# TIERS/multi-modal-loam

Measured on AMD Instinct MI355X. Metric: scans/s (feature-extract+kNN+10 GN iters) on 16-ring x1800 + Livox 24k fused cloud, higher is better.
Workload: dtype f32/f64; 1 GPU; BASELINE configs[1]: fused VLP-16 16x1800 + Livox Horizon 24000 scan (52800 pts), local map 200000 pts, 1 association pass (thres_dist 25), 10 GN iterations, W=1; resident_slots=8192, stream_lanes=2, distinct_scans=64, map_tiles_touched=43, map_tiles_complete=43, parallelism=scan-sharded x1, device=AMD Radeon Graphics, cus=256

## Files before the change

### multi-modal-loam_amd/csrc/capi.hip

```cpp
#include <math.h>
#include <stdarg.h>
#include <stdio.h>
#include <stdlib.h>
#include <string.h>

#include <algorithm>

#include "mml_internal.h"

int mml_launch_detect_line(mml_ctx* ctx, int n, uint16_t* d_final);

namespace {

constexpr int kPackMaxSlots = 16;
constexpr size_t kStageDoubles = 1u << 22;

double* stage_alloc(mml_ctx* ctx, size_t doubles) {
    if (ctx->stage_cursor + doubles > ctx->h_stage_doubles) {
        mml_sync_all(ctx);
        ctx->stage_cursor = 0;
    }
    double* p = ctx->h_stage + ctx->stage_cursor;
    ctx->stage_cursor += (doubles + 7) & ~size_t(7);
    return p;
}

hipError_t read_settings(mml_ctx* ctx) {
    hipDeviceProp_t prop;
    const hipError_t e = hipGetDeviceProperties(&prop, ctx->device);
    if (e != hipSuccess) return e;
    ctx->cus = prop.multiProcessorCount;
    ctx->n_lanes = 2;
    if (const char* v = getenv("MML_LANES")) {
        const int n = atoi(v);
        if (n >= 1 && n <= mml_ctx::MAX_LANES) ctx->n_lanes = n;
    }
    const auto off = [](const char* name) {
        const char* v = getenv(name);
        return v && atoi(v) == 0;
    };
    ctx->onepass_wanted = !off("MML_ASSIGN_ONEPASS");
    ctx->solve_wide = !off("MML_SOLVE_WIDE");
    ctx->use_graph = getenv("MML_NO_GRAPH") == nullptr;
    ctx->lazy_undistort = !off("MML_LAZY_UNDISTORT");
    return hipSuccess;
}

}

double* mml_stage_alloc(mml_ctx* ctx, size_t doubles) { return stage_alloc(ctx, doubles); }

int mml_refuse(mml_ctx* ctx, int code, const char* fmt, ...) {
    if (ctx) {
        char m[192];
        va_list ap;
        va_start(ap, fmt);
        vsnprintf(m, sizeof(m), fmt, ap);
        va_end(ap);
        ctx->err = m;
    }
    return code;
}

extern "C" {

void mml_config_default(mml_config* cfg, int max_scans) {
    memset(cfg, 0, sizeof(*cfg));
    cfg->max_scans = max_scans;
    cfg->max_velo_points = 16 * 1800;
    cfg->max_livox_points = 24000;
    cfg->n_rings = 16;
    cfg->pitch0_deg = -15.0f;
    cfg->pitch_step_deg = 2.0f;
    cfg->n_livox_lines = 6;
    cfg->near_th = 2.0f;
    cfg->far_th = 50.0f;
    cfg->leaf_corner = 0.4f;
// ... 109 lines not shown
    ALLOC(ctx->seg_flat_n, B * 4);
    ALLOC(ctx->op_agg, B * 2 * MML_SEG_MAX);
    ctx->seg_rstride = (int)((NT >> 6) + 6 * L + 8);
    ALLOC(ctx->seg_rs, B * (size_t)ctx->seg_rstride);
    ALLOC(ctx->seg_rw, B * (size_t)ctx->seg_rstride);
    ALLOC(ctx->ln_curv, B * NT);
    ALLOC(ctx->ln_refl, B * NT);
    ALLOC(ctx->ln_attr, B * NT);
    ALLOC(ctx->sel_scratch, 4 * B * NT + 16 * B * (L + 2) + 64);
    {
        const size_t nblk = ((NV > NL ? NV : NL) + 255) / 256;
        ALLOC(ctx->blk_cnt, B * 2 * nblk * 162);
    }
    ALLOC(ctx->assign_aux, B * 8);
    ALLOC(ctx->brk_queue, B * NT);
    ALLOC(ctx->brk_cnt, 2 * B);
    ALLOC(ctx->queue_off, 2 * ((size_t)B + mml_ctx::MAX_LANES + 1));
    ALLOC(ctx->redo_queue, B * NT);
    ALLOC(ctx->st_exit, B * (NT / 256 + L + 8));
    ALLOC(ctx->vx_big, 2 * B);
    ALLOC(ctx->sel_done, B * L + 8);
    ALLOC(ctx->sel_list, 4 * B * L + 8);
    ALLOC(ctx->sel_list_cnt, 2 * B + 8);
    ALLOC(ctx->crop_cnt, B * ((NT + 255) / 256) * 8);
    ALLOC(ctx->cb_n, B * 2);
    ALLOC(ctx->ln_line, B * NT);
    ALLOC(ctx->ln_label, B * NT);
    ALLOC(ctx->fu_info, B * 8);
    ALLOC(ctx->ft_xyz[0], B * MF);
    ALLOC(ctx->ft_xyz[1], B * MF);
    ALLOC(ctx->ft_n, B * 2);
    ALLOC(ctx->vx_keys, B * (size_t)ctx->VX_CAP);
    ALLOC(ctx->vx_gidx, 2 * B * (size_t)ctx->VX_CAP);
    ALLOC(ctx->lf, B * MF);
    ALLOC(ctx->pf, B * MF);
    ALLOC(ctx->assoc_stats, B * 16);
    ALLOC(ctx->hard_list, B * MF * 2);
    ALLOC(ctx->hard_knn, B * MF * 2 * 10);
    ALLOC(ctx->work_off, 2 * B + 8);
    for (int k = 0; k < 2; ++k) {
        ALLOC(ctx->grid[k].pts, MM);
        ALLOC(ctx->grid[k].cell_start, 4 * MM + 4096 + 2);
        ctx->grid[k].m = 0;
    }
    ALLOC(ctx->map_tmp, 2 * MM);
    ALLOC(ctx->map_keys, MM);
    ALLOC(ctx->map_keys2, MM);
    ALLOC(ctx->map_vals, MM);
    ALLOC(ctx->map_vals2, MM);
    ALLOC(ctx->d_x, B * 6);
    ALLOC(ctx->d_pose_in, B * 64);
    ALLOC(ctx->d_result, B * MML_SOLVE_RESULT);
    ALLOC(ctx->d_summ, B * 8);
    ALLOC(ctx->d_trace, B * 6 * 64);
    ALLOC(ctx->d_rec, B * 32);
    ALLOC(ctx->d_und, B * 8);
    ALLOC(ctx->d_und_par, B * 12);
    ALLOC(ctx->d_extr, 16);
    ALLOC(ctx->d_misc, 64);
#undef ALLOC
    ctx->h_stage_doubles = kStageDoubles;
    if ((e = ctx->fixed.alloc_pinned(&ctx->h_stage, ctx->h_stage_doubles + 8)) != hipSuccess) return fail(e, "ctx->h_stage");
    ctx->stage_cursor = 0;
    if (mml_feature_init(ctx) != MML_OK) return fail(hipErrorUnknown, "mml_feature_init");
    if ((e = hipStreamSynchronize(MML_STREAM(ctx))) != hipSuccess) return fail(e, "hipStreamSynchronize");
    *out = ctx;
// ... 714 lines not shown
    for (int i = 0; i < n; ++i) {
        if (lab[i] == 2) flat[nf++] = i;
        if (lab[i] == 1) sharp[ns++] = i;
        if (flags) flags[i] = fin[i];
    }
    *n_sharp = ns;
    *n_flat = nf;
    return MML_OK;
}

static int undistort_enqueue(mml_ctx* ctx, int first_slot, int count, const double* dR, const double* dt, bool listed_only) {
    double* st = stage_alloc(ctx, 12 * (size_t)count);
    for (int i = 0; i < count; ++i) {
        memcpy(st + 12 * i, dR + 9 * i, sizeof(double) * 9);
        memcpy(st + 12 * i + 9, dt + 3 * i, sizeof(double) * 3);
    }
    double* d_par = ctx->d_pose_in + 64 * (size_t)first_slot;
    MML_HIP(hipMemcpyAsync(d_par, st, sizeof(double) * 12 * count, hipMemcpyHostToDevice, MML_STREAM(ctx)));
    return listed_only ? mml_launch_undistort_listed(ctx, first_slot, count, d_par) : mml_launch_undistort(ctx, first_slot, count, d_par);
}

int mml_undistort(mml_ctx* ctx, int first_slot, int count, const double* dR, const double* dt) {
    CHECK_SLOTS(first_slot, count);
    MML_REQUIRE(dR && dt, MML_ERR_INVALID, "null dR/dt");
    int rc = mml_cloud_settle(ctx, first_slot, count);
    if (rc != MML_OK) return rc;
    return undistort_enqueue(ctx, first_slot, count, dR, dt, false);
}

int mml_downsample(mml_ctx* ctx, int first_slot, int count) {
    CHECK_SLOTS(first_slot, count);
    int rc = mml_cloud_settle(ctx, first_slot, count);
    if (rc != MML_OK) return rc;
    rc = mml_launch_downsample(ctx, first_slot, count);
    if (rc != MML_OK) return rc;
    return mml_downsample_redo_overflow(ctx, first_slot, count, nullptr);
}

int mml_features_download(mml_ctx* ctx, int slot, int kind, float* xyz, int capacity, int* n) {
    CHECK_SLOTS(slot, 1);
    MML_REQUIRE((kind == 0 || kind == 1) && n, MML_ERR_INVALID, "bad kind");
    int h = 0;
    MML_HIP(hipMemcpyAsync(&h, ctx->ft_n + kind * ctx->B + slot, sizeof(int), hipMemcpyDeviceToHost, MML_STREAM(ctx)));
    MML_HIP(hipStreamSynchronize(MML_STREAM(ctx)));
    MML_REQUIRE(h >= 0, MML_ERR_CAPACITY, "down-sample overflowed max_features / voxel capacity");
    *n = h;
    if (!xyz || h == 0) return MML_OK;
    MML_REQUIRE(capacity >= h, MML_ERR_CAPACITY, "download capacity too small");
    std::vector<float4> tmp(h);
    MML_HIP(hipMemcpyAsync(tmp.data(), ctx->ft_xyz[kind] + (size_t)slot * ctx->MF, sizeof(float4) * h,
                           hipMemcpyDeviceToHost, MML_STREAM(ctx)));
    MML_HIP(hipStreamSynchronize(MML_STREAM(ctx)));
    for (int i = 0; i < h; ++i) {
        xyz[3 * i] = tmp[i].x;
        xyz[3 * i + 1] = tmp[i].y;
        xyz[3 * i + 2] = tmp[i].z;
    }
    return MML_OK;
}

int mml_features_upload(mml_ctx* ctx, int slot, int kind, const float* xyz, int n) {
    CHECK_SLOTS(slot, 1);
    MML_REQUIRE((kind == 0 || kind == 1) && n >= 0 && (n == 0 || xyz), MML_ERR_INVALID, "bad arguments");
    MML_REQUIRE(n <= ctx->MF, MML_ERR_CAPACITY, "more features than max_features");
    std::vector<float4> tmp(n ? n : 1);
    for (int i = 0; i < n; ++i) tmp[i] = make_float4(xyz[3 * i], xyz[3 * i + 1], xyz[3 * i + 2], 0.f);
    if (n)
// ... 581 lines not shown
    if (packed) {
        const size_t c = (size_t)count, n = 34 * c + 16;
        double* hp = stage_alloc(ctx, n);
        dp = ctx->d_pose_in + 64 * (size_t)first_slot;
        for (size_t i = 0; i < c; ++i) {
            memcpy(hp + 12 * i, dR + 9 * i, sizeof(double) * 9);
            memcpy(hp + 12 * i + 9, dt + 3 * i, sizeof(double) * 3);
            double q[4];
            so3_exp_h(x_inout + 6 * i + 3, q);
            pose_to_Twl(q, x_inout + 6 * i, T_bl, hp + 12 * c + 16 * i);
        }
        memcpy(hp + 28 * c, x_inout, sizeof(double) * 6 * c);
        memcpy(hp + 34 * c, T_bl, sizeof(double) * 16);
        if (hipMemcpyAsync(dp, hp, sizeof(double) * n, hipMemcpyHostToDevice, MML_STREAM(ctx)) != hipSuccess) return MML_ERR_HIP;
        h_res = stage_alloc(ctx, MML_SOLVE_RESULT * c);
    }
    if (lanes > 1) {
        if (hipEventRecord(ctx->lane_mark[0], ctx->streams[0]) != hipSuccess) return MML_ERR_HIP;
        for (int l = 1; l < mml_ctx::MAX_LANES; ++l)
            if (hipStreamWaitEvent(ctx->streams[l], ctx->lane_mark[0], 0) != hipSuccess) return MML_ERR_HIP;
    }
    auto piece_span = [&](int p, int& f, int& c) {
        f = first_slot + p * chunk;
        c = std::min(chunk, first_slot + count - f);
        return c > 0;
    };
    auto run_stage = [&](int stage, int f, int c) -> int {
        const int off = f - first_slot;
        switch (stage) {
            case 0: return mml_launch_extract(ctx, f, c, false);
            case 1:
                if (packed) return ctx->lazy_undistort ? mml_launch_undistort_listed(ctx, f, c, dp) : mml_launch_undistort(ctx, f, c, dp);
                return undistort_enqueue(ctx, f, c, dR + 9 * (size_t)off, dt + 3 * (size_t)off, ctx->lazy_undistort);
            case 2: return mml_launch_downsample(ctx, f, c);
            case 3:
                if (packed) return mml_launch_associate(ctx, f, c, dp + 12 * (size_t)count, thres_dist, false);
                for (int i = 0; i < c; ++i) {
                    double q[4];
                    so3_exp_h(x_inout + 6 * (size_t)(off + i) + 3, q);
                    pose_to_Twl(q, x_inout + 6 * (size_t)(off + i), T_bl, &Twl[16 * (size_t)i]);
                }
                return associate_enqueue(ctx, f, c, Twl.data(), thres_dist, false);
            default: {
                if (packed) {
                    int r = mml_launch_solve(ctx, f, c, 1, dp + 34 * (size_t)count, so, false, dp + 28 * (size_t)count,
                                             ctx->d_result + MML_SOLVE_RESULT * (size_t)f);
                    if (r != MML_OK) return r;
                    if (hipMemcpyAsync(h_res, ctx->d_result + MML_SOLVE_RESULT * (size_t)f, sizeof(double) * MML_SOLVE_RESULT * c,
                                       hipMemcpyDeviceToHost, MML_STREAM(ctx)) != hipSuccess)
                        return MML_ERR_HIP;
                    return MML_OK;
                }
                int r = solve_enqueue(ctx, f, c, 1, T_bl, &so, x_inout + 6 * (size_t)off, false);
                if (r != MML_OK) return r;
                hipError_t e = hipMemcpyAsync(h_x + 6 * (size_t)off, ctx->d_x + 6 * (size_t)f, sizeof(double) * 6 * c, hipMemcpyDeviceToHost,
                                              MML_STREAM(ctx));
                if (e != hipSuccess) {
                    ctx->err = std::string("mml_step read-back: ") + hipGetErrorString(e);
                    return MML_ERR_HIP;
                }
                return MML_OK;
            }
        }
    };
    {
        for (int stage = 0; stage < 5 && rc == MML_OK; ++stage) {
            for (int l = 0; l < n_pieces && rc == MML_OK; ++l) {
// ... 343 lines not shown
```

### multi-modal-loam_amd/csrc/mml_internal.h

```cpp
#ifndef MML_INTERNAL_H
#define MML_INTERNAL_H

#include <hip/hip_runtime.h>
#include <stdint.h>

#include <string>
#include <vector>

#include "mml_mem.h"
#include "mmloam_hip.h"

#define MML_WAVE 64

namespace mml_und {
__device__ __forceinline__ double sconst(double v) {
    asm("" : "+s"(v));
    return v;
}
}
#define MML_SEG_MAX 16
#define MML_OP_BLK 4096
#define MML_SEG_FLAT 512
#define MML_VOXEL_LDS_CAP 8192

// ... 37 lines not shown
struct MmlLioDev;
struct MmlGicpDev;
struct MmlTofsDev;
struct MmlUnionDev;

struct mml_ctx {
    mml_config cfg;
    MmlComm* comm = nullptr;
    MmlFwDev* fwdev = nullptr;
    MmlPreintDev* preint = nullptr;
    MmlLioDev* lio = nullptr;
    MmlGicpDev* gicp = nullptr;
    MmlTofsDev* tofs = nullptr;
    MmlUnionDev* uni = nullptr;
    void* wstate = nullptr;
    double* wrec = nullptr;
    double* waux = nullptr;
    MmlGroup win_state;
    struct WinGraph {
        int first, count, W, max_iters, fixed;
        double huber, w_tan;
        hipStream_t stream;
        const double* Tbl;
        bool second;
        hipGraphExec_t exec;
    };
    std::vector<WinGraph> win_graphs;
    int device = 0;
    int cus = 0;
    bool onepass_wanted = true;
    bool solve_wide = true;
    bool use_graph = true;
    bool lazy_undistort = true;
    static constexpr int MAX_LANES = 8;
    hipStream_t streams[MAX_LANES] = {};
    hipStream_t copy_stream = nullptr;
    hipEvent_t lane_mark[MAX_LANES] = {};
    struct Upload {
        int first, count;
        hipEvent_t done;
    };
    std::vector<Upload> uploads;
    std::vector<hipEvent_t> upload_event_pool;
    int n_lanes = 1;
    int cur = 0;
    std::string err;
    MmlFixed fixed;

    int B = 0, NV = 0, NL = 0, NT = 0, L = 0, MF = 0;

    float4* velo_in = nullptr;
    mml_livox_point* livox_in = nullptr;
    int* d_n_in = nullptr;
    std::vector<int> h_n_in;
    std::vector<char> stats_stale;
    std::vector<char> raw_extracted;

    uint8_t* raw_line = nullptr;
    float* raw_ori = nullptr;

    float4* ln_pts = nullptr;
    int* ln_gidx = nullptr;
    int* ln_rel = nullptr;
    int* line_start = nullptr;
    int* line_len = nullptr;
    int* seg_cum = nullptr;
// ... 8 lines not shown
    unsigned op_epoch = 0;
    bool onepass = false;
    float* ln_curv = nullptr;
    float* ln_refl = nullptr;
    uint16_t* ln_attr = nullptr;
    int* crop_cnt = nullptr;
    int* blk_cnt = nullptr;
    int* assign_aux = nullptr;
    unsigned* sel_scratch = nullptr;
    int sel_cap = 0;
    int sel_cap_velo = 0;
    unsigned* brk_queue = nullptr;
    int* brk_cnt = nullptr;
    int* queue_off = nullptr;
    unsigned* redo_queue = nullptr;
    uint8_t* sel_done = nullptr;
    int* sel_list = nullptr;
    int* sel_list_cnt = nullptr;
    unsigned char* st_exit = nullptr;
    int* vx_big = nullptr;

    int* cb_n = nullptr;

    uint8_t* ln_line = nullptr;
    int* slot_flags = nullptr;
    std::vector<char> und_pending;
    uint8_t* ln_label = nullptr;
    int* fu_info = nullptr;

    float4* ft_xyz[2] = {nullptr, nullptr};
    int* ft_n = nullptr;
    unsigned long long* vx_keys = nullptr;
    int* vx_gidx = nullptr;
    unsigned long long* seg_keys = nullptr;
    unsigned* seg_vals = nullptr;
    float4* seg_cat = nullptr;
    int* seg_flag = nullptr;
    int* seg_meta = nullptr;
    MmlGroup seg_scratch;
    MmlStaging<char, false> seg_tmp[8];
    int VX_CAP = 0;

    MmlLineFactor* lf = nullptr;
    MmlPlaneFactor* pf = nullptr;
    int* work_off = nullptr;
    float* hard_knn = nullptr;
    int4* hard_list = nullptr;
    double* assoc_stats = nullptr;

    MmlGrid grid[2];
    bool have_map[2] = {false, false};
    MmlGrid ggrid[2];
    bool have_gmap[2] = {false, false};
    float4* gmap_orig[2] = {nullptr, nullptr};
    uint16_t* gtag_orig[2] = {nullptr, nullptr};
    int* cube_cnt[2] = {nullptr, nullptr};
    MmlGroup ggrid_mem[2];
    int gmap_cap[2] = {0, 0};
    int cen[3] = {10, 5, 10};
    static constexpr int LOCAL_WINDOW = 50;
    float4* ring[2] = {nullptr, nullptr};
    float4* ring_cat = nullptr;
    int* vox_flag = nullptr;
    size_t vox_cap = 0;
    MmlGroup ring_mem;
    int ring_n[2][LOCAL_WINDOW] = {};
// ... 73 lines not shown
        if (e_ != hipSuccess) {                                                               \
            ctx->err = std::string(#call) + ": " + hipGetErrorString(e_);                     \
            return MML_ERR_HIP;                                                               \
        }                                                                                     \
    } while (0)

#define MML_REQUIRE(cond, code, msg) \
    do {                             \
        if (!(cond)) {               \
            ctx->err = (msg);        \
            return (code);           \
        }                            \
    } while (0)

int mml_refuse(mml_ctx* ctx, int code, const char* fmt, ...) __attribute__((format(printf, 3, 4)));

inline int mml_sort_tmp(mml_ctx* ctx, size_t need) { return ctx->sort_tmp.reserve(ctx, need, MML_STREAM(ctx)); }

int mml_stage_begin(mml_ctx* ctx, const char* name);
void mml_stage_end(mml_ctx* ctx, int token);
struct MmlStageScope {
    mml_ctx* c;
    int t;
    MmlStageScope(mml_ctx* ctx, const char* name) : c(ctx), t(mml_stage_begin(ctx, name)) {}
    ~MmlStageScope() { mml_stage_end(c, t); }
};

int mml_launch_extract(mml_ctx* ctx, int first, int count, bool have_extrinsic);
int mml_launch_cloud_decode(mml_ctx* ctx, int slot, const float* d_raw, int n, int n_velo);
int mml_launch_undistort(mml_ctx* ctx, int first, int count, const double* d_params);
int mml_launch_undistort_listed(mml_ctx* ctx, int first, int count, const double* d_params);
int mml_cloud_settle(mml_ctx* ctx, int first, int count);
#define MML_LABEL_SETTLED 0x40
int mml_launch_downsample(mml_ctx* ctx, int first, int count);
inline int mml_voxel_cap_corner(const mml_ctx* ctx) { return (ctx->NT > 65536 || MML_VOXEL_LDS_CAP < 2048) ? MML_VOXEL_LDS_CAP : 2048; }
int mml_build_grid(mml_ctx* ctx, int kind, const float* h_xyz, int m);
int mml_build_grid_device(mml_ctx* ctx, int kind, int m);
int mml_downsample_big(mml_ctx* ctx, int first, int count);
int mml_downsample_redo_overflow(mml_ctx* ctx, int first, int count, std::vector<int>* redone);
int mml_map_upkeep_increment(mml_ctx* ctx, int slot, const double* T_wl, int* n_out);
int mml_build_global_grid(mml_ctx* ctx, int kind, const float* h_xyz, const int* h_cube, int m, const int* cen);
int mml_build_global_grid_device(mml_ctx* ctx, int kind, const float4* d_pts, const uint16_t* d_tags, const int* d_cnt, int m,
                                 const int* cen);
int mml_cube_store_append(mml_ctx* ctx, int slot, const double* T_wl);
int mml_cube_store_increment(mml_ctx* ctx, const double* T_wl, int* n_out);
int mml_cube_store_download(mml_ctx* ctx, int kind, float* xyz, int* cube, int capacity, int* n, int* cen);
int mml_cube_store_reset(mml_ctx* ctx);
int mml_launch_knn5(mml_ctx* ctx, int kind, const float* d_q, int nq, float max_d2, int* d_idx, float* d_d2);
int mml_launch_associate(mml_ctx* ctx, int first, int count, const double* d_Twl, double thres_dist, bool with_stats = true);
int mml_ensure_assoc_stats(mml_ctx* ctx, int first, int count);
#define MML_SOLVE_RESULT 24
int mml_launch_solve(mml_ctx* ctx, int first, int count, int window, const double* d_Tbl, mml_solve_opts opts,
                     bool want_trace, const double* d_x_in = nullptr, double* d_result = nullptr);
int mml_window_solve_continue(mml_ctx* ctx, int first, int count, int window, const double* d_Tbl, mml_solve_opts opts);
int mml_feature_init(mml_ctx* ctx);
void mml_fullwindow_dev_release(mml_ctx* ctx);
void mml_imu_preint_release(mml_ctx* ctx);
void mml_lio_init_release(mml_ctx* ctx);
void mml_gicp_release(mml_ctx* ctx);
void mml_time_offset_release(mml_ctx* ctx);
void mml_union_release(mml_ctx* ctx);
int mml_union_check(mml_ctx* ctx, mml_livox_stream* s, int first_slot, int count, const uint64_t* stamps, const float* velo_xyzi,
                    const int* velo_offsets, mml_union_frame* out);
int mml_union_run(mml_ctx* ctx, mml_livox_stream* s, int first_slot, int count, const uint64_t* stamps, const float* velo_xyzi,
                  const int* velo_offsets, const float* tf, mml_union_frame* out);
int mml_launch_detect_line(mml_ctx* ctx, int n, uint16_t* d_final);
int mml_launch_raw_lines(mml_ctx* ctx, int first, int count);
int mml_launch_linearize(mml_ctx* ctx, int slot, const double* d_x, const double* d_Tbl, double w_tan,
// ... 4 lines not shown
```

### multi-modal-loam_amd/csrc/undistort_voxel.hip

```cpp
#include <math.h>

#include "mml_internal.h"
#include "undistort_dev.h"

namespace {
using namespace mml_und;

__global__ void k_undistort_prep(int count, const double* params, double* derived, double* par_keep, int* flags ) {
    const int s = blockIdx.x * blockDim.x + threadIdx.x;
    if (s >= count) return;
    for (int k = 0; k < 12; ++k) par_keep[12 * s + k] = params[12 * s + k];
    flags[2 * s + 1] = flags[2 * s];
    flags[2 * s] |= 2;
    const double* dR = params + 12 * s;
    const Q4 qlc = qnormalized(quat_from_matrix(dR));
    const double dd = (0.0 * qlc.x + 0.0 * qlc.z) + (0.0 * qlc.y + 1.0 * qlc.w);
    const double absD = fabs(dd);
    const double one = 1.0 - 2.220446049250313e-16;
    double theta = 0, sinTheta = 1;
    const bool linear = absD >= one;
    if (!linear) {
        theta = acos(absD);
        sinTheta = sin(theta);
    }
// ... 19 lines not shown
    if constexpr (SETTLE) {
        uint8_t* lab = ln_label + (size_t)b * NT + i;
        const unsigned l = *lab;
        if (l & MML_LABEL_SETTLED) {
            *lab = (uint8_t)(l & ~(unsigned)MML_LABEL_SETTLED);
            return;
        }
    }
    const double* dR = params + 12 * blockIdx.y;
    typedef float v4f __attribute__((ext_vector_type(4)));
    v4f* pp = reinterpret_cast<v4f*>(ln_pts + (size_t)b * NT + i);
    const v4f raw = __builtin_nontemporal_load(pp);
    float4 p = make_float4(raw.x, raw.y, raw.z, raw.w);
    const float s = (slot_flags[2 * b + 1] & 2) ? 1.0f : __int_as_float(__builtin_nontemporal_load(&ln_rel[(size_t)b * NT + i]));
    mml_und::undistort_point(dR, dR + 9, derived + 8 * blockIdx.y, s, p);
    v4f outv = {p.x, p.y, p.z, p.w};
    __builtin_nontemporal_store(outv, pp);
}

constexpr int UND_LISTED_G = 8;
__device__ __forceinline__ int listed_position(const int* fu_info, const unsigned* lists, int list_stride, int NT, int b, int e) {
    const int nc = min(max(fu_info[8 * b + 6], 0), list_stride), ns = min(max(fu_info[8 * b + 7], 0), list_stride);
    if (e >= nc + ns) return -1;
    const int kind = e >= nc ? 1 : 0;
    const unsigned pos = lists[((size_t)b * 2 + kind) * list_stride + (e - (kind ? nc : 0))];
    return pos < (unsigned)NT ? (int)pos : -1;
}
__device__ __forceinline__ int listed_total(const int* fu_info, int list_stride, int b) {
    return min(max(fu_info[8 * b + 6], 0), list_stride) + min(max(fu_info[8 * b + 7], 0), list_stride);
}

__global__ __launch_bounds__(256) void k_undistort_listed(int first, int NT, int list_stride, const int* fu_info, const unsigned* lists,
                                                         float4* ln_pts, const int* ln_rel, const int* slot_flags, const double* params,
                                                         const double* derived) {
    const int b = blockIdx.y + first;
    const int n = listed_total(fu_info, list_stride, b);
    const bool time_is_one = (slot_flags[2 * b + 1] & 2) != 0;
    const double* dR = params + 12 * blockIdx.y;
    for (int e = blockIdx.x * 256 + threadIdx.x; e < n; e += UND_LISTED_G * 256) {
        const int pos = listed_position(fu_info, lists, list_stride, NT, b, e);
        if (pos < 0) continue;
        float4 p = ln_pts[(size_t)b * NT + pos];
        const float s = time_is_one ? 1.0f : __int_as_float(ln_rel[(size_t)b * NT + pos]);
        mml_und::undistort_point(dR, dR + 9, derived + 8 * blockIdx.y, s, p);
        ln_pts[(size_t)b * NT + pos] = p;
    }
}

__global__ __launch_bounds__(256) void k_settle_mark(int first, int NT, int list_stride, const int* fu_info, const unsigned* lists,
                                                    uint8_t* ln_label) {
    const int b = blockIdx.y + first;
    const int n = listed_total(fu_info, list_stride, b);
    for (int e = blockIdx.x * 256 + threadIdx.x; e < n; e += UND_LISTED_G * 256) {
        const int pos = listed_position(fu_info, lists, list_stride, NT, b, e);
        if (pos < 0) continue;
        uint8_t* lab = ln_label + (size_t)b * NT + pos;
        *lab = (uint8_t)(*lab | MML_LABEL_SETTLED);
    }
}

#ifdef MML_VX_TIMING
__device__ unsigned long long g_vx_dbg[16];
#define VX_MARK(id)                                    \
    do {                                               \
        if (vx_dbg) {                                  \
            const unsigned long long now_ = clock64(); \
            g_vx_dbg[id] += now_ - vx_prev;            \
            vx_prev = now_;                            \
        }                                              \
    } while (0)
extern "C" int mml_debug_vx_timing(unsigned long long* out, int reset) {
    if (reset) {
        unsigned long long z[16] = {};
        return hipMemcpyToSymbol(HIP_SYMBOL(g_vx_dbg), z, sizeof(z)) == hipSuccess ? 0 : -1;
    }
    return hipMemcpyFromSymbol(out, HIP_SYMBOL(g_vx_dbg), sizeof(unsigned long long) * 16) == hipSuccess ? 0 : -1;
}
#define VX_DBG_PARAMS , bool vx_dbg, unsigned long long& vx_prev
// ... 97 lines not shown
            for (int w = 0; w < wave; ++w) base += wtot[w];
#pragma unroll
            for (int q = 0; q < PER; ++q) {
                const int idx = PER * tid + q, d = idx / VX_WAVES, w = idx % VX_WAVES;
                hist[w * 256 + d] = (unsigned short)base;
                base += c[q];
            }
        }
        __syncthreads();
#pragma unroll
        for (int a = 0; a < KPT; ++a) {
            const int e = (wave * KPT + a) * 64 + lane;
            if (e < cnt) lds[(int)hist[wave * 256 + (rd[a] >> 16)] + (int)(rd[a] & 0xffffu)] = key[a];
        }
        in_lds = true;
    }
    if (!in_lds) {
#pragma unroll
        for (int a = 0; a < KPT; ++a) {
            const int e = (wave * KPT + a) * 64 + lane;
            if (e < cnt) lds[e] = key[a];
        }
    }
    __syncthreads();
}

struct VoxelArgs {
    int kind0, first, NT, MF, B, cap_y0, cap_y1, list_stride;
    int skip_above, only_above;
    int zero_big;
    int* big;
    const int* fu_info;
    const float4* ln_pts;
    const int* ln_gidx;
    float leaf_corner, leaf_surf;
    float4* ft0;
    float4* ft1;
    int* ft_n;
    const unsigned* seq_scratch;
    const int* seq_gidx;
};
template <int VX_THREADS>
struct VoxelLds {
    static constexpr int VX_WAVES = VX_THREADS / 64;
    union {
        float stage[3][VX_THREADS + VX_TAIL];
        unsigned short hist[VX_WAVES * 256];
    } u;
    int wtot[VX_WAVES + 2];
    unsigned long long red[2 * VX_WAVES];
    float red6[6][VX_WAVES];
    int base, nout;
};

template <int VX_THREADS, int KPT>
__device__ __forceinline__ void voxel_sort(const VoxelArgs& A, VoxelLds<VX_THREADS>& S, unsigned long long* keys, int b, int kind, int cnt,
                                           const unsigned* seq2idx, const float4* px, const int* glist, bool wide, float leaf VX_DBG_PARAMS) {
    constexpr int VX_WAVES = VX_THREADS / 64;
    const int tid = threadIdx.x, lane = tid & 63, wave = tid >> 6;
    constexpr bool KEEP = KPT <= 4;
    constexpr int KR = KEEP ? KPT : 1;
    unsigned pos[KPT];
    float x[KR], y[KR], z[KR];
    int gi[KR];
#pragma unroll
    for (int a = 0; a < KPT; ++a) pos[a] = seq2idx[min((wave * KPT + a) * 64 + lane, cnt - 1)];
    float mn[3] = {INFINITY, INFINITY, INFINITY}, mx[3] = {-INFINITY, -INFINITY, -INFINITY};
#pragma unroll
    for (int a0 = 0; a0 < KPT; a0 += 4) {
        float4 p4[4];
#pragma unroll
        for (int a = a0; a < a0 + 4 && a < KPT; ++a) p4[a - a0] = px[pos[a]];
#pragma unroll
        for (int a = a0; a < a0 + 4 && a < KPT; ++a) {
            const float4 p = p4[a - a0];
            if constexpr (KEEP) {
                x[a] = p.x;
                y[a] = p.y;
                z[a] = p.z;
                gi[a] = glist[min((wave * KPT + a) * 64 + lane, cnt - 1)];
            }
            mn[0] = fminf(mn[0], p.x);
            mn[1] = fminf(mn[1], p.y);
            mn[2] = fminf(mn[2], p.z);
            mx[0] = fmaxf(mx[0], p.x);
            mx[1] = fmaxf(mx[1], p.y);
            mx[2] = fmaxf(mx[2], p.z);
        }
        __builtin_amdgcn_sched_barrier(0);
    }
    VX_MARK(4);
    float gmn[3], gmx[3];
#pragma unroll
    for (int c = 0; c < 3; ++c) {
        for (int o = 32; o > 0; o >>= 1) {
            mn[c] = fminf(mn[c], __shfl_xor(mn[c], o));
            mx[c] = fmaxf(mx[c], __shfl_xor(mx[c], o));
        }
        if (lane == 0) {
            S.red6[c][wave] = mn[c];
            S.red6[3 + c][wave] = mx[c];
        }
    }
    __syncthreads();
#pragma unroll
    for (int c = 0; c < 3; ++c) {
        float r0 = S.red6[c][0], r1 = S.red6[3 + c][0];
        for (int w = 1; w < VX_WAVES; ++w) {
            r0 = fminf(r0, S.red6[c][w]);
            r1 = fmaxf(r1, S.red6[3 + c][w]);
        }
        gmn[c] = r0;
        gmx[c] = r1;
    }
    VX_MARK(5);
    const float inv = 1.0f / leaf;
    int min_b[3], div_b[3];
    for (int c = 0; c < 3; ++c) {
        min_b[c] = static_cast<int>(floor(gmn[c] * inv));
        const int max_b = static_cast<int>(floor(gmx[c] * inv));
        div_b[c] = max_b - min_b[c] + 1;
    }
    const int mul1 = div_b[0], mul2 = div_b[0] * div_b[1];
    const bool unfiltered = mml_voxel_grid_overflows(gmn, gmx, inv);
    unsigned long long key[KPT];
#pragma unroll
    for (int a = 0; a < KPT; ++a) {
        const int sidx = (wave * KPT + a) * 64 + lane;
        float px_, py_, pz_;
        int g;
        if constexpr (KEEP) {
            px_ = x[a];
            py_ = y[a];
            pz_ = z[a];
            g = gi[a];
        } else {
            const float4 p = px[pos[a]];
            px_ = p.x;
            py_ = p.y;
            pz_ = p.z;
            g = glist[min(sidx, cnt - 1)];
        }
        const int ijk0 = static_cast<int>(floor(px_ * inv) - static_cast<float>(min_b[0]));
        const int ijk1 = static_cast<int>(floor(py_ * inv) - static_cast<float>(min_b[1]));
        const int ijk2 = static_cast<int>(floor(pz_ * inv) - static_cast<float>(min_b[2]));
        const int idx = unfiltered ? g : ijk0 + ijk1 * mul1 + ijk2 * mul2;
        key[a] = wide ? (((unsigned long long)(unsigned)idx << 33) | ((unsigned long long)(unsigned)g << 13) | (unsigned)sidx)
                      : (((unsigned long long)(unsigned)idx << 32) | ((unsigned)g << 16) | pos[a]);
    }
    VX_MARK(6);
    radix_sort_lds<VX_THREADS, KPT>(key, cnt, wide ? 13 : 16, keys, S.u.hist, S.wtot, S.red VX_DBG_ARGS);
    VX_MARK(7);
}

#ifndef MML_VOXEL_WAVES
#define MML_VOXEL_WAVES 8
#endif
template <int VX_THREADS>
__device__ __forceinline__ void voxel_slot(const VoxelArgs& A, VoxelLds<VX_THREADS>& S, unsigned long long* keys, int b, int kind, int cap) {
    constexpr int VX_WAVES = VX_THREADS / 64;
    const int tid = threadIdx.x, lane = tid & 63, wave = tid >> 6;
    const int NT = A.NT, MF = A.MF;
    const float4* px = A.ln_pts + (size_t)b * NT;
    const float leaf = kind == 0 ? A.leaf_corner : A.leaf_surf;
    float4* out = (kind == 0 ? A.ft0 : A.ft1) + (size_t)b * MF;
    const unsigned* seq2idx = A.seq_scratch + ((size_t)b * 2 + kind) * A.list_stride;
    const int* glist = A.seq_gidx + ((size_t)b * 2 + kind) * A.list_stride;
    const unsigned long long lt = (lane == 0) ? 0ull : (~0ull >> (64 - lane));
    static_assert(MML_VOXEL_LDS_CAP <= 8192, "the wide key layout carries the place in the label list in 13 bits");
    const bool wide = NT > 65536;
    const int vshift = wide ? 33 : 32;
    auto key_pos = [&](unsigned long long k) -> unsigned { return wide ? seq2idx[(unsigned)k & 0x1fffu] : (unsigned)k & 0xffffu; };

#ifdef MML_VX_TIMING
    const bool vx_dbg = tid == 64 && kind == MML_VX_TIMING && blockIdx.x == 517 && VX_THREADS == 512;
    unsigned long long vx_prev = clock64();
#endif
    const int nsel = A.fu_info[8 * b + 6 + kind];
    if (A.skip_above > 0 && nsel > A.skip_above) {
        if (tid == 0) A.big[A.B + A.first + atomicAdd(&A.big[A.first], 1)] = b;
        return;
    }
    const int cnt = nsel > cap ? cap : nsel;
    const bool overflow = nsel > cap;
    if (cnt == 0) {
        if (tid == 0) A.ft_n[kind * A.B + b] = 0;
        return;
    }
    if (cnt <= VX_THREADS)
        voxel_sort<VX_THREADS, 1>(A, S, keys, b, kind, cnt, seq2idx, px, glist, wide, leaf VX_DBG_ARGS);
    else if (cnt <= 2 * VX_THREADS)
        voxel_sort<VX_THREADS, 2>(A, S, keys, b, kind, cnt, seq2idx, px, glist, wide, leaf VX_DBG_ARGS);
    else if (cnt <= 4 * VX_THREADS)
        voxel_sort<VX_THREADS, 4>(A, S, keys, b, kind, cnt, seq2idx, px, glist, wide, leaf VX_DBG_ARGS);
    else
        voxel_sort<VX_THREADS, 8>(A, S, keys, b, kind, cnt, seq2idx, px, glist, wide, leaf VX_DBG_ARGS);
    VX_MARK(0);
    if (tid == 0) {
        S.base = 0;
        S.nout = 0;
    }
    __syncthreads();
    for (int c0 = 0; c0 < cnt; c0 += VX_THREADS) {
        const int s = c0 + tid;
        bool head = false;
        unsigned vox = 0;
        if (s < cnt) {
            vox = (unsigned)(keys[s] >> vshift);
            head = (s == 0) || ((unsigned)(keys[s - 1] >> vshift) != vox);
        }
        for (int t = tid; t < VX_THREADS + VX_TAIL; t += VX_THREADS) {
            const int e = c0 + t;
            if (e < cnt) {
                const float4 p = px[key_pos(keys[e])];
                S.u.stage[0][t] = p.x;
                S.u.stage[1][t] = p.y;
                S.u.stage[2][t] = p.z;
            }
        }
        unsigned long long m = __ballot(head);
        if (lane == 0) S.wtot[wave] = __popcll(m);
        __syncthreads();
        VX_MARK(1);
        int dst = S.base;
        for (int w = 0; w < wave; ++w) dst += S.wtot[w];
        dst += __popcll(m & lt);
        if (head && dst < MF) {
            float sx = 0, sy = 0, sz = 0;
            int e = s;
            while (e < cnt && (unsigned)(keys[e] >> vshift) == vox) {
                const int t = e - c0;
                if (t < VX_THREADS + VX_TAIL) {
                    sx += S.u.stage[0][t];
                    sy += S.u.stage[1][t];
                    sz += S.u.stage[2][t];
                } else {
                    const float4 p = px[key_pos(keys[e])];
                    sx += p.x;
                    sy += p.y;
                    sz += p.z;
                }
                ++e;
            }
            float c = static_cast<float>(e - s);
            out[dst] = make_float4(sx / c, sy / c, sz / c, 0.f);
        }
        VX_MARK(2);
        __syncthreads();
        VX_MARK(3);
        if (tid == 0) {
            int t = 0;
            for (int w = 0; w < VX_WAVES; ++w) t += S.wtot[w];
            S.base += t;
        }
        __syncthreads();
    }
    if (tid == 0) {
        int nout = S.base;
        if (overflow || nout > MF) nout = -1;
        A.ft_n[kind * A.B + b] = nout;
    }
}
template <int VX_THREADS, bool LIST = false>
__global__ __launch_bounds__(VX_THREADS) __attribute__((amdgpu_waves_per_eu(MML_VOXEL_WAVES))) void k_voxel(VoxelArgs A) {
    extern __shared__ __attribute__((aligned(16))) unsigned char smem[];
    unsigned long long* keys = reinterpret_cast<unsigned long long*>(smem);
    __shared__ VoxelLds<VX_THREADS> S;
    const int kind = blockIdx.y + A.kind0;
    const int cap = blockIdx.y == 0 ? A.cap_y0 : A.cap_y1;
    if constexpr (LIST) {
        const int nbig = A.big[A.first];
        for (int e = blockIdx.x; e < nbig; e += gridDim.x) {
            voxel_slot<VX_THREADS>(A, S, keys, __builtin_amdgcn_readfirstlane(A.big[A.B + A.first + e]), kind, cap);
            __syncthreads();
        }
    } else {
        if (A.zero_big && blockIdx.x == 0 && blockIdx.y == 0 && threadIdx.x == 0) A.big[A.first] = 0;
        voxel_slot<VX_THREADS>(A, S, keys, (int)blockIdx.x + A.first, kind, cap);
    }
}

}

int mml_launch_undistort(mml_ctx* ctx, int first, int count, const double* d_params) {
    MmlStageScope t(ctx, "undistort");
    dim3 grid((ctx->NT + 255) / 256, count);
    hipLaunchKernelGGL(k_undistort_prep, dim3((count + 63) / 64), dim3(64), 0, MML_STREAM(ctx), count, d_params, ctx->d_und + 8 * (size_t)first,
                       ctx->d_und_par + 12 * (size_t)first, ctx->slot_flags + 2 * (size_t)first);
    hipLaunchKernelGGL(k_undistort<false>, grid, dim3(256), 0, MML_STREAM(ctx), first, ctx->NT, ctx->NV, ctx->cb_n, ctx->ln_pts,
                       ctx->ln_rel, ctx->slot_flags, d_params, ctx->d_und + 8 * (size_t)first, (uint8_t*)nullptr);
    MML_HIP(hipGetLastError());
    return MML_OK;
}

int mml_launch_undistort_listed(mml_ctx* ctx, int first, int count, const double* d_params) {
    MmlStageScope t(ctx, "undistort");
    for (int i = 0; i < count; ++i) ctx->und_pending[first + i] = 1;
    hipLaunchKernelGGL(k_undistort_prep, dim3((count + 63) / 64), dim3(64), 0, MML_STREAM(ctx), count, d_params, ctx->d_und + 8 * (size_t)first,
                       ctx->d_und_par + 12 * (size_t)first, ctx->slot_flags + 2 * (size_t)first);
    hipLaunchKernelGGL(k_undistort_listed, dim3(UND_LISTED_G, count), dim3(256), 0, MML_STREAM(ctx), first, ctx->NT, ctx->VX_CAP, ctx->fu_info,
                       reinterpret_cast<const unsigned*>(ctx->vx_keys), ctx->ln_pts, ctx->ln_rel, ctx->slot_flags, d_params,
                       ctx->d_und + 8 * (size_t)first);
    MML_HIP(hipGetLastError());
    return MML_OK;
}

int mml_cloud_settle(mml_ctx* ctx, int first, int count) {
    for (int i = 0; i < count;) {
        if (!ctx->und_pending[first + i]) {
            ++i;
            continue;
        }
        int n = 1;
        while (i + n < count && ctx->und_pending[first + i + n] && n < 32768) ++n;
        const int f = first + i;
        MmlStageScope t(ctx, "undistort_settle");
        hipLaunchKernelGGL(k_settle_mark, dim3(UND_LISTED_G, n), dim3(256), 0, MML_STREAM(ctx), f, ctx->NT, ctx->VX_CAP, ctx->fu_info,
                           reinterpret_cast<const unsigned*>(ctx->vx_keys), ctx->ln_label);
        hipLaunchKernelGGL(k_undistort<true>, dim3((ctx->NT + 255) / 256, n), dim3(256), 0, MML_STREAM(ctx), f, ctx->NT, ctx->NV, ctx->cb_n,
                           ctx->ln_pts, ctx->ln_rel, ctx->slot_flags, ctx->d_und_par + 12 * (size_t)f, ctx->d_und + 8 * (size_t)f, ctx->ln_label);
        MML_HIP(hipGetLastError());
        for (int k = 0; k < n; ++k) ctx->und_pending[f + k] = 0;
        i += n;
    }
    return MML_OK;
}

int mml_launch_downsample(mml_ctx* ctx, int first, int count) {
    MmlStageScope t(ctx, "voxel_downsample");
    for (int i = 0; i < count; ++i) ctx->stats_stale[first + i] = 1;
    if (ctx->NT > (1 << 20)) return mml_downsample_big(ctx, first, count);
    const int cap_surf = MML_VOXEL_LDS_CAP, cap_corner = mml_voxel_cap_corner(ctx);
    auto lds = [](int cap) { return (size_t)cap * sizeof(unsigned long long); };
    VoxelArgs A;
    A.first = first;
    A.NT = ctx->NT;
    A.MF = ctx->MF;
    A.B = ctx->B;
    A.list_stride = ctx->VX_CAP;
    A.fu_info = ctx->fu_info;
    A.ln_pts = ctx->ln_pts;
    A.ln_gidx = ctx->ln_gidx;
    A.leaf_corner = ctx->cfg.leaf_corner;
    A.leaf_surf = ctx->cfg.leaf_surf;
    A.ft0 = ctx->ft_xyz[0];
    A.ft1 = ctx->ft_xyz[1];
    A.ft_n = ctx->ft_n;
    A.seq_scratch = reinterpret_cast<const unsigned*>(ctx->vx_keys);
    A.seq_gidx = ctx->vx_gidx;
    A.skip_above = 0;
    A.only_above = 0;
    A.zero_big = 0;
    A.big = ctx->vx_big;
    if (cap_corner == cap_surf || count <= 16) {
        A.kind0 = 0;
        A.cap_y0 = cap_corner;
        A.cap_y1 = cap_surf;
        hipLaunchKernelGGL(k_voxel<1024>, dim3(count, 2), dim3(1024), lds(cap_surf), MML_STREAM(ctx), A);
    } else {
        A.kind0 = 0;
        A.cap_y0 = A.cap_y1 = cap_corner;
        A.zero_big = 1;
        hipLaunchKernelGGL(k_voxel<256>, dim3(count, 1), dim3(256), lds(cap_corner), MML_STREAM(ctx), A);
        A.zero_big = 0;
        constexpr int cap_mid = 4096;
        static_assert(cap_mid < MML_VOXEL_LDS_CAP, "the 512-thread form takes the short lists only");
        A.kind0 = 1;
        A.cap_y0 = A.cap_y1 = cap_mid;
        A.skip_above = cap_mid;
        hipLaunchKernelGGL(k_voxel<512>, dim3(count, 1), dim3(512), lds(cap_mid), MML_STREAM(ctx), A);
        A.cap_y0 = A.cap_y1 = cap_surf;
        A.skip_above = 0;
        A.only_above = cap_mid;
        hipLaunchKernelGGL((k_voxel<1024, true>), dim3(count < 256 ? count : 256, 1), dim3(1024), lds(cap_surf), MML_STREAM(ctx), A);
    }
    MML_HIP(hipGetLastError());
    return MML_OK;
}
```

Measured before the change: 444,500 scans/s.

## Write undistorted feature points into packed per-slot buffer for voxel downsample

The listed undistort kernel now also writes each undistorted point into a compact per-slot buffer ordered by label-list position, with corner points first and surface points after a fixed offset. The 256- and 512-thread voxel kernels read from this packed buffer directly instead of gathering through the seq2idx indirection into the full ln_pts array. The goal is to remove a dependent indirect load and scattered global reads during the voxel sort. The cost is an extra buffer allocation and extra stores in the undistort kernel, and the path only applies when the corner cap differs from the LDS cap and more than 16 slots are processed.

```diff
diff --git a/multi-modal-loam_amd/csrc/capi.hip b/multi-modal-loam_amd/csrc/capi.hip
--- a/multi-modal-loam_amd/csrc/capi.hip
+++ b/multi-modal-loam_amd/csrc/capi.hip
@@ -43,6 +43,7 @@
     ctx->solve_wide = !off("MML_SOLVE_WIDE");
     ctx->use_graph = getenv("MML_NO_GRAPH") == nullptr;
     ctx->lazy_undistort = !off("MML_LAZY_UNDISTORT");
+    ctx->voxel_packed = !off("MML_VOXEL_PACKED");
     return hipSuccess;
 }
 
@@ -218,6 +219,9 @@
     ALLOC(ctx->ft_n, B * 2);
     ALLOC(ctx->vx_keys, B * (size_t)ctx->VX_CAP);
     ALLOC(ctx->vx_gidx, 2 * B * (size_t)ctx->VX_CAP);
+    if (ctx->voxel_packed && ctx->lazy_undistort && mml_voxel_cap_corner(ctx) != MML_VOXEL_LDS_CAP) {
+        ALLOC(ctx->vx_pts, B * (size_t)mml_voxel_packed_stride(ctx));
+    }
     ALLOC(ctx->lf, B * MF);
     ALLOC(ctx->pf, B * MF);
     ALLOC(ctx->assoc_stats, B * 16);
@@ -998,7 +1002,7 @@
     CHECK_SLOTS(first_slot, count);
     int rc = mml_cloud_settle(ctx, first_slot, count);
     if (rc != MML_OK) return rc;
-    rc = mml_launch_downsample(ctx, first_slot, count);
+    rc = mml_launch_downsample(ctx, first_slot, count, false);
     if (rc != MML_OK) return rc;
     return mml_downsample_redo_overflow(ctx, first_slot, count, nullptr);
 }
@@ -1646,7 +1650,8 @@
             case 1:
                 if (packed) return ctx->lazy_undistort ? mml_launch_undistort_listed(ctx, f, c, dp) : mml_launch_undistort(ctx, f, c, dp);
                 return undistort_enqueue(ctx, f, c, dR + 9 * (size_t)off, dt + 3 * (size_t)off, ctx->lazy_undistort);
-            case 2: return mml_launch_downsample(ctx, f, c);
+            case 2:
+                return mml_launch_downsample(ctx, f, c, mml_voxel_step_packed(ctx, c));
             case 3:
                 if (packed) return mml_launch_associate(ctx, f, c, dp + 12 * (size_t)count, thres_dist, false);
                 for (int i = 0; i < c; ++i) {
diff --git a/multi-modal-loam_amd/csrc/mml_internal.h b/multi-modal-loam_amd/csrc/mml_internal.h
--- a/multi-modal-loam_amd/csrc/mml_internal.h
+++ b/multi-modal-loam_amd/csrc/mml_internal.h
@@ -93,6 +93,7 @@
     bool solve_wide = true;
     bool use_graph = true;
     bool lazy_undistort = true;
+    bool voxel_packed = true;
     static constexpr int MAX_LANES = 8;
     hipStream_t streams[MAX_LANES] = {};
     hipStream_t copy_stream = nullptr;
@@ -167,6 +168,7 @@
     int* ft_n = nullptr;
     unsigned long long* vx_keys = nullptr;
     int* vx_gidx = nullptr;
+    float4* vx_pts = nullptr;
     unsigned long long* seg_keys = nullptr;
     unsigned* seg_vals = nullptr;
     float4* seg_cat = nullptr;
@@ -306,8 +308,10 @@
 int mml_launch_undistort_listed(mml_ctx* ctx, int first, int count, const double* d_params);
 int mml_cloud_settle(mml_ctx* ctx, int first, int count);
 #define MML_LABEL_SETTLED 0x40
-int mml_launch_downsample(mml_ctx* ctx, int first, int count);
+int mml_launch_downsample(mml_ctx* ctx, int first, int count, bool packed);
 inline int mml_voxel_cap_corner(const mml_ctx* ctx) { return (ctx->NT > 65536 || MML_VOXEL_LDS_CAP < 2048) ? MML_VOXEL_LDS_CAP : 2048; }
+inline int mml_voxel_packed_stride(const mml_ctx* ctx) { return mml_voxel_cap_corner(ctx) + MML_VOXEL_LDS_CAP; }
+bool mml_voxel_step_packed(const mml_ctx* ctx, int count);
 int mml_build_grid(mml_ctx* ctx, int kind, const float* h_xyz, int m);
 int mml_build_grid_device(mml_ctx* ctx, int kind, int m);
 int mml_downsample_big(mml_ctx* ctx, int first, int count);
diff --git a/multi-modal-loam_amd/csrc/undistort_voxel.hip b/multi-modal-loam_amd/csrc/undistort_voxel.hip
--- a/multi-modal-loam_amd/csrc/undistort_voxel.hip
+++ b/multi-modal-loam_amd/csrc/undistort_voxel.hip
@@ -75,9 +75,10 @@
 
 __global__ __launch_bounds__(256) void k_undistort_listed(int first, int NT, int list_stride, const int* fu_info, const unsigned* lists,
                                                          float4* ln_pts, const int* ln_rel, const int* slot_flags, const double* params,
-                                                         const double* derived) {
+                                                         const double* derived, float4* packed, int packed_stride, int cap_corner) {
     const int b = blockIdx.y + first;
     const int n = listed_total(fu_info, list_stride, b);
+    const int nc = min(max(fu_info[8 * b + 6], 0), list_stride);
     const bool time_is_one = (slot_flags[2 * b + 1] & 2) != 0;
     const double* dR = params + 12 * blockIdx.y;
     for (int e = blockIdx.x * 256 + threadIdx.x; e < n; e += UND_LISTED_G * 256) {
@@ -87,6 +88,11 @@
         const float s = time_is_one ? 1.0f : __int_as_float(ln_rel[(size_t)b * NT + pos]);
         mml_und::undistort_point(dR, dR + 9, derived + 8 * blockIdx.y, s, p);
         ln_pts[(size_t)b * NT + pos] = p;
+        if (packed) {
+            const bool surf = e >= nc;
+            const int place = surf ? e - nc : e;
+            if (place < (surf ? MML_VOXEL_LDS_CAP : cap_corner)) packed[(size_t)b * packed_stride + (surf ? cap_corner : 0) + place] = p;
+        }
     }
 }
 
@@ -250,6 +256,8 @@
     int* big;
     const int* fu_info;
     const float4* ln_pts;
+    const float4* vx_pts;
+    int vx_stride, vx_corner;
     const int* ln_gidx;
     float leaf_corner, leaf_surf;
     float4* ft0;
@@ -271,24 +279,31 @@
     int base, nout;
 };
 
-template <int VX_THREADS, int KPT>
+template <int VX_THREADS, int KPT, bool PACKED>
 __device__ __forceinline__ void voxel_sort(const VoxelArgs& A, VoxelLds<VX_THREADS>& S, unsigned long long* keys, int b, int kind, int cnt,
                                            const unsigned* seq2idx, const float4* px, const int* glist, bool wide, float leaf VX_DBG_PARAMS) {
     constexpr int VX_WAVES = VX_THREADS / 64;
     const int tid = threadIdx.x, lane = tid & 63, wave = tid >> 6;
     constexpr bool KEEP = KPT <= 4;
     constexpr int KR = KEEP ? KPT : 1;
-    unsigned pos[KPT];
+    unsigned pos[PACKED ? 1 : KPT];
     float x[KR], y[KR], z[KR];
     int gi[KR];
-#pragma unroll
-    for (int a = 0; a < KPT; ++a) pos[a] = seq2idx[min((wave * KPT + a) * 64 + lane, cnt - 1)];
+    const int last = cnt - 1;
+    auto where = [&](int a) -> unsigned {
+        if constexpr (PACKED) return (unsigned)min((wave * KPT + a) * 64 + lane, last);
+        else return pos[a];
+    };
+    if constexpr (!PACKED) {
+#pragma unroll
+        for (int a = 0; a < KPT; ++a) pos[a] = seq2idx[min((wave * KPT + a) * 64 + lane, cnt - 1)];
+    }
     float mn[3] = {INFINITY, INFINITY, INFINITY}, mx[3] = {-INFINITY, -INFINITY, -INFINITY};
 #pragma unroll
     for (int a0 = 0; a0 < KPT; a0 += 4) {
         float4 p4[4];
 #pragma unroll
-        for (int a = a0; a < a0 + 4 && a < KPT; ++a) p4[a - a0] = px[pos[a]];
+        for (int a = a0; a < a0 + 4 && a < KPT; ++a) p4[a - a0] = px[where(a)];
 #pragma unroll
         for (int a = a0; a < a0 + 4 && a < KPT; ++a) {
             const float4 p = p4[a - a0];
@@ -353,7 +368,7 @@
             pz_ = z[a];
             g = gi[a];
         } else {
-            const float4 p = px[pos[a]];
+            const float4 p = px[where(a)];
             px_ = p.x;
             py_ = p.y;
             pz_ = p.z;
@@ -364,7 +379,7 @@
         const int ijk2 = static_cast<int>(floor(pz_ * inv) - static_cast<float>(min_b[2]));
         const int idx = unfiltered ? g : ijk0 + ijk1 * mul1 + ijk2 * mul2;
         key[a] = wide ? (((unsigned long long)(unsigned)idx << 33) | ((unsigned long long)(unsigned)g << 13) | (unsigned)sidx)
-                      : (((unsigned long long)(unsigned)idx << 32) | ((unsigned)g << 16) | pos[a]);
+                      : (((unsigned long long)(unsigned)idx << 32) | ((unsigned)g << 16) | (PACKED ? (unsigned)sidx : where(a)));
     }
     VX_MARK(6);
     radix_sort_lds<VX_THREADS, KPT>(key, cnt, wide ? 13 : 16, keys, S.u.hist, S.wtot, S.red VX_DBG_ARGS);
@@ -374,12 +389,12 @@
 #ifndef MML_VOXEL_WAVES
 #define MML_VOXEL_WAVES 8
 #endif
-template <int VX_THREADS>
+template <int VX_THREADS, bool PACKED>
 __device__ __forceinline__ void voxel_slot(const VoxelArgs& A, VoxelLds<VX_THREADS>& S, unsigned long long* keys, int b, int kind, int cap) {
     constexpr int VX_WAVES = VX_THREADS / 64;
     const int tid = threadIdx.x, lane = tid & 63, wave = tid >> 6;
     const int NT = A.NT, MF = A.MF;
-    const float4* px = A.ln_pts + (size_t)b * NT;
+    const float4* px = PACKED ? A.vx_pts + (size_t)b * A.vx_stride + (kind ? A.vx_corner : 0) : A.ln_pts + (size_t)b * NT;
     const float leaf = kind == 0 ? A.leaf_corner : A.leaf_surf;
     float4* out = (kind == 0 ? A.ft0 : A.ft1) + (size_t)b * MF;
     const unsigned* seq2idx = A.seq_scratch + ((size_t)b * 2 + kind) * A.list_stride;
@@ -388,7 +403,10 @@
     static_assert(MML_VOXEL_LDS_CAP <= 8192, "the wide key layout carries the place in the label list in 13 bits");
     const bool wide = NT > 65536;
     const int vshift = wide ? 33 : 32;
-    auto key_pos = [&](unsigned long long k) -> unsigned { return wide ? seq2idx[(unsigned)k & 0x1fffu] : (unsigned)k & 0xffffu; };
+    auto key_pos = [&](unsigned long long k) -> unsigned {
+        if constexpr (PACKED) return (unsigned)k & 0x1fffu;
+        return wide ? seq2idx[(unsigned)k & 0x1fffu] : (unsigned)k & 0xffffu;
+    };
 
 #ifdef MML_VX_TIMING
     const bool vx_dbg = tid == 64 && kind == MML_VX_TIMING && blockIdx.x == 517 && VX_THREADS == 512;
@@ -406,13 +424,13 @@
         return;
     }
     if (cnt <= VX_THREADS)
-        voxel_sort<VX_THREADS, 1>(A, S, keys, b, kind, cnt, seq2idx, px, glist, wide, leaf VX_DBG_ARGS);
+        voxel_sort<VX_THREADS, 1, PACKED>(A, S, keys, b, kind, cnt, seq2idx, px, glist, wide, leaf VX_DBG_ARGS);
     else if (cnt <= 2 * VX_THREADS)
-        voxel_sort<VX_THREADS, 2>(A, S, keys, b, kind, cnt, seq2idx, px, glist, wide, leaf VX_DBG_ARGS);
+        voxel_sort<VX_THREADS, 2, PACKED>(A, S, keys, b, kind, cnt, seq2idx, px, glist, wide, leaf VX_DBG_ARGS);
     else if (cnt <= 4 * VX_THREADS)
-        voxel_sort<VX_THREADS, 4>(A, S, keys, b, kind, cnt, seq2idx, px, glist, wide, leaf VX_DBG_ARGS);
+        voxel_sort<VX_THREADS, 4, PACKED>(A, S, keys, b, kind, cnt, seq2idx, px, glist, wide, leaf VX_DBG_ARGS);
     else
-        voxel_sort<VX_THREADS, 8>(A, S, keys, b, kind, cnt, seq2idx, px, glist, wide, leaf VX_DBG_ARGS);
+        voxel_sort<VX_THREADS, 8, PACKED>(A, S, keys, b, kind, cnt, seq2idx, px, glist, wide, leaf VX_DBG_ARGS);
     VX_MARK(0);
     if (tid == 0) {
         S.base = 0;
@@ -479,7 +497,7 @@
         A.ft_n[kind * A.B + b] = nout;
     }
 }
-template <int VX_THREADS, bool LIST = false>
+template <int VX_THREADS, bool LIST, bool PACKED>
 __global__ __launch_bounds__(VX_THREADS) __attribute__((amdgpu_waves_per_eu(MML_VOXEL_WAVES))) void k_voxel(VoxelArgs A) {
     extern __shared__ __attribute__((aligned(16))) unsigned char smem[];
     unsigned long long* keys = reinterpret_cast<unsigned long long*>(smem);
@@ -489,12 +507,12 @@
     if constexpr (LIST) {
         const int nbig = A.big[A.first];
         for (int e = blockIdx.x; e < nbig; e += gridDim.x) {
-            voxel_slot<VX_THREADS>(A, S, keys, __builtin_amdgcn_readfirstlane(A.big[A.B + A.first + e]), kind, cap);
+            voxel_slot<VX_THREADS, PACKED>(A, S, keys, __builtin_amdgcn_readfirstlane(A.big[A.B + A.first + e]), kind, cap);
             __syncthreads();
         }
     } else {
         if (A.zero_big && blockIdx.x == 0 && blockIdx.y == 0 && threadIdx.x == 0) A.big[A.first] = 0;
-        voxel_slot<VX_THREADS>(A, S, keys, (int)blockIdx.x + A.first, kind, cap);
+        voxel_slot<VX_THREADS, PACKED>(A, S, keys, (int)blockIdx.x + A.first, kind, cap);
     }
 }
 
@@ -518,7 +536,8 @@
                        ctx->d_und_par + 12 * (size_t)first, ctx->slot_flags + 2 * (size_t)first);
     hipLaunchKernelGGL(k_undistort_listed, dim3(UND_LISTED_G, count), dim3(256), 0, MML_STREAM(ctx), first, ctx->NT, ctx->VX_CAP, ctx->fu_info,
                        reinterpret_cast<const unsigned*>(ctx->vx_keys), ctx->ln_pts, ctx->ln_rel, ctx->slot_flags, d_params,
-                       ctx->d_und + 8 * (size_t)first);
+                       ctx->d_und + 8 * (size_t)first, mml_voxel_step_packed(ctx, count) ? ctx->vx_pts : (float4*)nullptr, mml_voxel_packed_stride(ctx),
+                       mml_voxel_cap_corner(ctx));
     MML_HIP(hipGetLastError());
     return MML_OK;
 }
@@ -544,7 +563,24 @@
     return MML_OK;
 }
 
-int mml_launch_downsample(mml_ctx* ctx, int first, int count) {
+namespace {
+template <int VX_THREADS, bool LIST>
+void launch_voxel(mml_ctx* ctx, bool packed, dim3 grid, size_t lds, const VoxelArgs& A) {
+    if constexpr (VX_THREADS <= 512 && !LIST) {
+        if (packed) {
+            hipLaunchKernelGGL((k_voxel<VX_THREADS, false, true>), grid, dim3(VX_THREADS), lds, MML_STREAM(ctx), A);
+            return;
+        }
+    }
+    hipLaunchKernelGGL((k_voxel<VX_THREADS, LIST, false>), grid, dim3(VX_THREADS), lds, MML_STREAM(ctx), A);
+}
+}
+
+bool mml_voxel_step_packed(const mml_ctx* ctx, int count) {
+    return ctx->vx_pts != nullptr && count > 16 && mml_voxel_cap_corner(ctx) != MML_VOXEL_LDS_CAP;
+}
+
+int mml_launch_downsample(mml_ctx* ctx, int first, int count, bool packed) {
     MmlStageScope t(ctx, "voxel_downsample");
     for (int i = 0; i < count; ++i) ctx->stats_stale[first + i] = 1;
     if (ctx->NT > (1 << 20)) return mml_downsample_big(ctx, first, count);
@@ -558,6 +594,9 @@
     A.list_stride = ctx->VX_CAP;
     A.fu_info = ctx->fu_info;
     A.ln_pts = ctx->ln_pts;
+    A.vx_pts = ctx->vx_pts;
+    A.vx_stride = mml_voxel_packed_stride(ctx);
+    A.vx_corner = cap_corner;
     A.ln_gidx = ctx->ln_gidx;
     A.leaf_corner = ctx->cfg.leaf_corner;
     A.leaf_surf = ctx->cfg.leaf_surf;
@@ -574,23 +613,23 @@
         A.kind0 = 0;
         A.cap_y0 = cap_corner;
         A.cap_y1 = cap_surf;
-        hipLaunchKernelGGL(k_voxel<1024>, dim3(count, 2), dim3(1024), lds(cap_surf), MML_STREAM(ctx), A);
+        launch_voxel<1024, false>(ctx, packed, dim3(count, 2), lds(cap_surf), A);
     } else {
         A.kind0 = 0;
         A.cap_y0 = A.cap_y1 = cap_corner;
         A.zero_big = 1;
-        hipLaunchKernelGGL(k_voxel<256>, dim3(count, 1), dim3(256), lds(cap_corner), MML_STREAM(ctx), A);
+        launch_voxel<256, false>(ctx, packed, dim3(count, 1), lds(cap_corner), A);
         A.zero_big = 0;
         constexpr int cap_mid = 4096;
         static_assert(cap_mid < MML_VOXEL_LDS_CAP, "the 512-thread form takes the short lists only");
         A.kind0 = 1;
         A.cap_y0 = A.cap_y1 = cap_mid;
         A.skip_above = cap_mid;
-        hipLaunchKernelGGL(k_voxel<512>, dim3(count, 1), dim3(512), lds(cap_mid), MML_STREAM(ctx), A);
+        launch_voxel<512, false>(ctx, packed, dim3(count, 1), lds(cap_mid), A);
         A.cap_y0 = A.cap_y1 = cap_surf;
         A.skip_above = 0;
         A.only_above = cap_mid;
-        hipLaunchKernelGGL((k_voxel<1024, true>), dim3(count < 256 ? count : 256, 1), dim3(1024), lds(cap_surf), MML_STREAM(ctx), A);
+        launch_voxel<1024, true>(ctx, packed, dim3(count < 256 ? count : 256, 1), lds(cap_surf), A);
     }
     MML_HIP(hipGetLastError());
     return MML_OK;
```

Result: faster. 448,900 scans/s (median of 6 runs) (+1.0%).
